# MichSchli/RelationPrediction

Hardware: AMD Instinct MI355X
Metric: processed edges/sec (R-GCN forward+backward), FB15k-237 gcn_block (higher is better)
Workload: dtype f32 (dense contractions: fp32 operands split exactly into 3 bf16, 6 of 9 partial products on the bf16 matrix cores, fp32 accumulation; error vs float64 equal to the fp32 MFMA's); 1 GPU; fb237_block; entities=14541, relations=237, dim=500, layers=2, kind=block, num_blocks_or_bases=100, graph_edges=15000, norm_mode=intended (1/deg of the edge's own row; SURVEY H1, DESIGN section 10), parallelism=single GPU

## Files before the change

### relationprediction_amd/csrc/block_msgs.hip

```cpp
#include <type_traits>

#include "rgcn_internal.h"

namespace rgcn {

namespace {

__device__ __forceinline__ int find_segment(const int32_t* __restrict__ ptr, int n_seg, int x) {
  int lo = 0, hi = n_seg;
  while (hi - lo > 1) {
    int mid = (lo + hi) >> 1;
    if (ptr[mid] <= x) lo = mid; else hi = mid;
  }
  return lo;
}

struct MsgArgs {
  const float* Hin;
  const float* D;
  const float* W;
  float* out;
  float* slab;
  const int32_t* m_src;
  const int32_t* m_dst;
  const int32_t* m_slot;
  const float* m_norm;
  const int32_t* rel_ptr;
  const int32_t* chunk_ptr;
  int32_t R2, nb, d, chunk, G;
};

template <int SD>
__global__ void k_block_msg_fwd(MsgArgs a) {
  const int bid = blockIdx.x;
  if (bid >= a.chunk_ptr[a.R2]) return;
  const int g = threadIdx.x / a.nb;
  if (g >= a.G) return;
  const int b = threadIdx.x - g * a.nb;
  const int rel = find_segment(a.chunk_ptr, a.R2, bid);
  const int beg = a.rel_ptr[rel] + (bid - a.chunk_ptr[rel]) * a.chunk;
  const int end = min(beg + a.chunk, a.rel_ptr[rel + 1]);
  float w[SD * SD];
#pragma unroll
  for (int k = 0; k < SD * SD; ++k) w[k] = a.W[((size_t)rel * SD * SD + k) * a.nb + b];
  const int col = b * SD;
// ... 4 lines not shown
    const float* xp = a.Hin + (size_t)src * a.d + col;
    float x[SD];
#pragma unroll
    for (int q = 0; q < SD; ++q) x[q] = xp[q];
    float* yp = a.out + (size_t)slot * a.d + col;
#pragma unroll
    for (int i = 0; i < SD; ++i) {
      float y = 0.0f;
#pragma unroll
      for (int q = 0; q < SD; ++q) y = fmaf(w[i * SD + q], x[q], y);
      yp[i] = y * nrm;
    }
  }
}

template <int SD, bool ZOUT>
__global__ void k_block_msg_bwd(MsgArgs a) {
  extern __shared__ float red[];
  const int bid = blockIdx.x;
  if (bid >= a.chunk_ptr[a.R2]) return;
  const int g = threadIdx.x / a.nb;
  const bool active = g < a.G;
  const int b = threadIdx.x - g * a.nb;
  const int rel = find_segment(a.chunk_ptr, a.R2, bid);
  const int beg = a.rel_ptr[rel] + (bid - a.chunk_ptr[rel]) * a.chunk;
  const int end = min(beg + a.chunk, a.rel_ptr[rel + 1]);
  float w[SD * SD], dw[SD * SD];
#pragma unroll
  for (int k = 0; k < SD * SD; ++k) dw[k] = 0.0f;
  if (active) {
    if constexpr (ZOUT) {
#pragma unroll
      for (int k = 0; k < SD * SD; ++k) w[k] = a.W[((size_t)rel * SD * SD + k) * a.nb + b];
    }
    const int col = b * SD;
    for (int j = beg + g; j < end; j += a.G) {
      const int src = a.m_src[j];
      const int dst = a.m_dst[j];
      const int slot = ZOUT ? a.m_slot[j] : 0;
      const float nrm = a.m_norm[j];
      const float* xp = a.Hin + (size_t)src * a.d + col;
      const float* gp = a.D + (size_t)dst * a.d + col;
      float x[SD], gr[SD];
#pragma unroll
      for (int q = 0; q < SD; ++q) { x[q] = xp[q]; gr[q] = gp[q] * nrm; }
      if constexpr (ZOUT) {
        float* zp = a.out + (size_t)slot * a.d + col;
#pragma unroll
        for (int q = 0; q < SD; ++q) {
          float z = 0.0f;
#pragma unroll
          for (int i = 0; i < SD; ++i) z = fmaf(w[i * SD + q], gr[i], z);
          zp[q] = z;
        }
      }
#pragma unroll
      for (int i = 0; i < SD; ++i)
#pragma unroll
        for (int q = 0; q < SD; ++q) dw[i * SD + q] = fmaf(gr[i], x[q], dw[i * SD + q]);
    }
  }
  if (a.G > 1) {
    if (active && g > 0) {
#pragma unroll
      for (int k = 0; k < SD * SD; ++k) red[((size_t)(g - 1) * SD * SD + k) * a.nb + b] = dw[k];
    }
    __syncthreads();
    if (active && g == 0) {
      for (int gg = 1; gg < a.G; ++gg)
#pragma unroll
        for (int k = 0; k < SD * SD; ++k) dw[k] += red[((size_t)(gg - 1) * SD * SD + k) * a.nb + b];
    }
  }
  if (active && g == 0) {
#pragma unroll
    for (int k = 0; k < SD * SD; ++k) a.slab[((size_t)bid * SD * SD + k) * a.nb + b] = dw[k];
  }
}

__global__ void k_block_dw_reduce(const float* __restrict__ slab, const int32_t* __restrict__ chunk_ptr,
                                  float* __restrict__ gW, int R2, int per_rel) {
  const int64_t i = (int64_t)blockIdx.x * blockDim.x + threadIdx.x;
  if (i >= (int64_t)R2 * per_rel) return;
  const int rel = (int)(i / per_rel);
  const int k = (int)(i - (int64_t)rel * per_rel);
  const int c0 = chunk_ptr[rel], c1 = chunk_ptr[rel + 1];
  float a0 = 0.f, a1 = 0.f, a2 = 0.f, a3 = 0.f, a4 = 0.f, a5 = 0.f, a6 = 0.f, a7 = 0.f;
  int c = c0;
  for (; c + 8 <= c1; c += 8) {
    const float* p = slab + (size_t)c * per_rel + k;
    a0 += p[0]; a1 += p[(size_t)per_rel]; a2 += p[2 * (size_t)per_rel]; a3 += p[3 * (size_t)per_rel];
    a4 += p[4 * (size_t)per_rel]; a5 += p[5 * (size_t)per_rel]; a6 += p[6 * (size_t)per_rel];
    a7 += p[7 * (size_t)per_rel];
  }
  for (; c < c1; ++c) a0 += slab[(size_t)c * per_rel + k];
  gW[i] = ((a0 + a1) + (a2 + a3)) + ((a4 + a5) + (a6 + a7));
}

__global__ void k_block_transpose(const float* __restrict__ in, float* __restrict__ out, int R, int nb,
                                  int sd2, int to_device) {
  const int64_t i = (int64_t)blockIdx.x * blockDim.x + threadIdx.x;
  const int64_t n = (int64_t)R * nb * sd2;
  if (i >= n) return;
  const int b = (int)(i % nb);
  const int k = (int)((i / nb) % sd2);
  const int r = (int)(i / ((int64_t)nb * sd2));
  const int64_t h = ((int64_t)r * nb + b) * sd2 + k;
  if (to_device) out[i] = in[h]; else out[h] = in[i];
}

int max_chunks(const rgcn_ctx* c) {
// ... 45 lines not shown
  a.rel_ptr = c->g.rel_ptr; a.chunk_ptr = c->g.chunk_ptr;
  a.R2 = 2 * c->R; a.nb = c->nb; a.d = c->d; a.chunk = c->g.chunk; a.G = c->msg_slots;
  const double M = 2.0 * c->g.E / c->world;
  const double rows = M < c->V ? M : (double)c->V;
  const double Wb = 8.0 * c->R * c->nb * c->sd * c->sd;
  ProfScope ps(c, "block_msg_fwd", M * (8.0 * c->d + 16.0) + Wb, M * 2.0 * c->d * c->sd,
               4.0 * c->d * (rows + M) + 16.0 * M + Wb);
  RGCN_TRY(dispatch_sd(c, [&](auto sdc) {
    constexpr int SD = decltype(sdc)::value;
    hipLaunchKernelGGL((k_block_msg_fwd<SD>), dim3(max_chunks(c)), dim3(c->msg_block), 0, c->stream, a);
  }));
  RGCN_HIP(c, hipGetLastError());
  return RGCN_OK;
}

rgcn_status block_msg_backward(rgcn_ctx* c, int layer, const float* Hin, const float* D, float* Zbuf) {
  const int per_rel = c->sd * c->sd * c->nb;
  const int R2 = 2 * c->R;
  if (c->g.E > 0) {
    const int nchunks = max_chunks(c);
    if ((size_t)nchunks * per_rel > c->slab_dw_floats)
      RGCN_FAIL(c, RGCN_ERR_STATE, "internal: dW slab buffer too small");
    MsgArgs a;
    a.Hin = Hin; a.D = D; a.W = c->layers[layer].wrel; a.out = Zbuf; a.slab = c->slab_dw;
    a.m_src = c->g.m_src; a.m_dst = c->g.m_dst; a.m_slot = c->g.m_sslot; a.m_norm = c->g.m_norm;
    a.rel_ptr = c->g.rel_ptr; a.chunk_ptr = c->g.chunk_ptr;
    a.R2 = R2; a.nb = c->nb; a.d = c->d; a.chunk = c->g.chunk; a.G = c->msg_slots;
    const size_t lds = (size_t)(c->msg_slots - 1) * per_rel * sizeof(float);
    const double M = 2.0 * c->g.E / c->world;
    const double rows = M < c->V ? M : (double)c->V;
    if (Zbuf != nullptr) {
      ProfScope ps(c, "block_msg_bwd", M * (12.0 * c->d + 20.0) + 16.0 * c->R * per_rel,
                   M * 4.0 * c->d * c->sd, 4.0 * c->d * (2.0 * rows + M) + 20.0 * M + 16.0 * c->R * per_rel);
      RGCN_TRY(dispatch_sd(c, [&](auto sdc) {
        constexpr int SD = decltype(sdc)::value;
        hipLaunchKernelGGL((k_block_msg_bwd<SD, true>), dim3(nchunks), dim3(c->msg_block), lds, c->stream, a);
      }));
    } else {
      ProfScope ps(c, "block_dw_msgs", M * (8.0 * c->d + 16.0) + 8.0 * c->R * per_rel, M * 2.0 * c->d * c->sd,
                   4.0 * c->d * 2.0 * rows + 16.0 * M + 8.0 * c->R * per_rel);
      RGCN_TRY(dispatch_sd(c, [&](auto sdc) {
        constexpr int SD = decltype(sdc)::value;
        hipLaunchKernelGGL((k_block_msg_bwd<SD, false>), dim3(nchunks), dim3(c->msg_block), lds, c->stream, a);
      }));
    }
    RGCN_HIP(c, hipGetLastError());
  }
  return RGCN_OK;
}

rgcn_status block_dw_reduce(rgcn_ctx* c, int layer) {
  const int per_rel = c->sd * c->sd * c->nb;
  const int R2 = 2 * c->R;
  {
    const int64_t n = (int64_t)R2 * per_rel;
    ProfScope ps(c, "block_dw_reduce", 8.0 * n, 0);
    hipLaunchKernelGGL(k_block_dw_reduce, dim3((unsigned)((n + 255) / 256)), dim3(256), 0, c->stream,
                       c->slab_dw, c->g.chunk_ptr, c->layers[layer].grel, R2, per_rel);
    RGCN_HIP(c, hipGetLastError());
  }
  return RGCN_OK;
}

rgcn_status block_to_device_layout(rgcn_ctx* c, const float* host_layout_dev, float* dst, int R) {
  const int64_t n = (int64_t)R * c->nb * c->sd * c->sd;
  hipLaunchKernelGGL(k_block_transpose, dim3((unsigned)((n + 255) / 256)), dim3(256), 0, c->stream,
                     host_layout_dev, dst, R, c->nb, c->sd * c->sd, 1);
  RGCN_HIP(c, hipGetLastError());
  return RGCN_OK;
}

rgcn_status block_from_device_layout(rgcn_ctx* c, const float* src, float* host_layout_dev, int R) {
  const int64_t n = (int64_t)R * c->nb * c->sd * c->sd;
  hipLaunchKernelGGL(k_block_transpose, dim3((unsigned)((n + 255) / 256)), dim3(256), 0, c->stream,
                     src, host_layout_dev, R, c->nb, c->sd * c->sd, 0);
// ... 6 lines not shown
```

### relationprediction_amd/csrc/graph_prep.hip

```cpp
#include "rgcn_internal.h"

namespace rgcn {

namespace {

constexpr int kScanThreads = 1024;
constexpr int kScanItems = 16;

struct ScanJob {
  const int32_t* in;
  int32_t* out;
  int32_t n;
  int32_t div;
  int32_t* where;
};
struct ScanJobs {
  ScanJob j[5];
};

__global__ void __launch_bounds__(kScanThreads) k_exscan(ScanJobs jobs) {
  const ScanJob job = jobs.j[blockIdx.x];
  __shared__ int32_t wsum[kScanThreads / 64];
  __shared__ int32_t carry_s;
  const int tid = threadIdx.x, lane = tid & 63, wid = tid >> 6;
// ... 66 lines not shown
}

__device__ __forceinline__ int lower_bound_u32(const uint32_t* a, int n, uint32_t x) {
  int lo = 0, hi = n;
  while (lo < hi) {
    int mid = (lo + hi) >> 1;
    if (a[mid] < x) lo = mid + 1; else hi = mid;
  }
  return lo;
}

__global__ void __launch_bounds__(1024) k_ptrs(const uint32_t* __restrict__ keyv_s,
                                               const uint32_t* __restrict__ keyr_s,
                                               const int32_t* __restrict__ permv, int E, int degrees_from_rows,
                                               int32_t* indeg, int32_t* outdeg, int M, int V, int R2,
                                               int chunk, int32_t* row_ptr,
                                               int32_t* long_rows, int32_t* nlong, int cap, int giant_threshold,
                                               int32_t* giant_rows, int32_t* giant_first, int32_t* giant_cnt,
                                               int32_t* piece_row, int32_t* piece_k, int32_t* ngiant, int giant_cap,
                                               int piece_cap, int32_t* rel_ptr, int32_t* chunk_ptr,
                                               uint32_t* row_key, int32_t* has_dir, uint32_t vmul) {
  if (blockIdx.x == 0) {
    __shared__ int32_t wsum[16];
    __shared__ int32_t carry_s;
    const int tid = threadIdx.x, lane = tid & 63, wid = tid >> 6;
    if (tid == 0) carry_s = 0;
    __syncthreads();
    for (int base = 0; base <= R2; base += 1024) {
      const int r = base + tid;
      int lo = 0, nchunks = 0;
      if (r <= R2) {
        lo = lower_bound_u32(keyr_s, M, (uint32_t)r);
        rel_ptr[r] = lo;
        if (r < R2) {
          const int hi = lower_bound_u32(keyr_s, M, (uint32_t)(r + 1));
          nchunks = (hi - lo + chunk - 1) / chunk;
        }
      }
      int incl = nchunks;
#pragma unroll
      for (int off = 1; off < 64; off <<= 1) {
        int t = __shfl_up(incl, off, 64);
        if (lane >= off) incl += t;
      }
      if (lane == 63) wsum[wid] = incl;
      __syncthreads();
      int wbase = 0, total = 0;
      for (int w = 0; w < 16; ++w) {
        if (w < wid) wbase += wsum[w];
        total += wsum[w];
      }
      const int carry = carry_s;
      if (r <= R2) chunk_ptr[r] = carry + wbase + incl - nchunks;
      __syncthreads();
      if (tid == 0) carry_s = carry + total;
      __syncthreads();
    }
    return;
  }
  const int v = (blockIdx.x - 1) * blockDim.x + threadIdx.x;
  if (v > V) return;
  const int beg = lower_bound_u32(keyv_s, M, (uint32_t)v * vmul);
  row_ptr[v] = beg;
  if (v == V) return;
  const int end = lower_bound_u32(keyv_s, M, (uint32_t)(v + 1) * vmul);
  if (row_key != nullptr) row_key[v] = end - beg > kLongRow ? (uint32_t)(kLongRow + 1) : (uint32_t)(kLongRow - (end - beg));
  if (degrees_from_rows || has_dir != nullptr) {
    int lo = beg, hi = end;
    while (lo < hi) {
      const int mid = (lo + hi) >> 1;
      if (permv[mid] < E) lo = mid + 1; else hi = mid;
// ... 226 lines not shown
  g.outdeg = g.counters + V;
  g.nlong = g.counters + 2 * V;
  g.ngiant = g.counters + 2 * V + 1;
  g.giant_cap = (int32_t)(M / kGiantRow + 1);
  g.piece_cap = (int32_t)(2 * (M / kGiantRow) + 2);
  RGCN_TRY(dalloc(c, &g.giant_rows, (size_t)g.giant_cap));
  RGCN_TRY(dalloc(c, &g.giant_first, (size_t)g.giant_cap));
  RGCN_TRY(dalloc(c, &g.giant_cnt, (size_t)g.giant_cap));
  RGCN_TRY(dalloc(c, &g.piece_row, (size_t)g.piece_cap));
  RGCN_TRY(dalloc(c, &g.piece_k, (size_t)g.piece_cap));
  g.long_cap = (int32_t)(M / kLongRow + 1);
  RGCN_TRY(dalloc(c, &g.long_rows, (size_t)g.long_cap));
  RGCN_TRY(dalloc(c, &g.row_ptr, V + 1));
  RGCN_TRY(dalloc(c, &g.rel_ptr, R2 + 1));
  RGCN_TRY(dalloc(c, &g.chunk_ptr, R2 + 1));
  RGCN_TRY(dalloc(c, &g.cum_in, V + 1));
  RGCN_TRY(dalloc(c, &g.cum_out, V + 1));
  RGCN_TRY(dalloc(c, &g.keyv, M));
  RGCN_TRY(dalloc(c, &g.keyv_s, M));
  RGCN_TRY(dalloc(c, &g.keyr, M));
  RGCN_TRY(dalloc(c, &g.keyr_s, M));
  RGCN_TRY(dalloc(c, &g.valv, M));
  RGCN_TRY(dalloc(c, &g.permv, M));
  RGCN_TRY(dalloc(c, &g.valr, M));
  RGCN_TRY(dalloc(c, &g.permr, M));
  RGCN_TRY(dalloc(c, &g.pos, M));
  RGCN_TRY(dalloc(c, &g.m_src, M));
  RGCN_TRY(dalloc(c, &g.m_dst, M));
  RGCN_TRY(dalloc(c, &g.m_dslot, M));
  RGCN_TRY(dalloc(c, &g.m_sslot, M));
// ... 20 lines not shown
  }
  if (share) {
    g.owner = share->owner;
    g.errflag = share->errflag;
  } else {
    RGCN_TRY(dalloc(c, &g.owner, (size_t)c->R));
    RGCN_TRY(dalloc(c, &g.errflag, 1));
    RGCN_HIP(c, hipMemsetAsync(g.owner, 0, sizeof(int32_t) * (size_t)(c->R ? c->R : 1), c->stream));
    RGCN_HIP(c, hipMemsetAsync(g.errflag, 0, sizeof(int32_t), c->stream));
  }
  RGCN_HIP(c, hipEventCreateWithFlags(&g.ev_ready, order_event_flags(c)));
  RGCN_HIP(c, hipEventCreateWithFlags(&g.ev_free, order_event_flags(c)));
  RGCN_HIP(c, hipMemsetAsync(g.row_ptr, 0, sizeof(int32_t) * (V + 1), c->stream));
  RGCN_HIP(c, hipMemsetAsync(g.rel_ptr, 0, sizeof(int32_t) * (R2 + 1), c->stream));
  RGCN_HIP(c, hipMemsetAsync(g.chunk_ptr, 0, sizeof(int32_t) * (R2 + 1), c->stream));
  RGCN_TRY(dalloc(c, &g.keyv_t, M));
  RGCN_TRY(dalloc(c, &g.keyr_t, M));
  RGCN_TRY(dalloc(c, &g.tablev, sort_table_elems(M)));
  RGCN_TRY(dalloc(c, &g.tabler, sort_table_elems(M)));
  return RGCN_OK;
}

static void graph_free_one(GraphBufs& g, bool owns_shared) {
  if (!owns_shared) { g.owner = nullptr; g.errflag = nullptr; }
  if (g.ev_ready) (void)hipEventDestroy(g.ev_ready);
  if (g.ev_free) (void)hipEventDestroy(g.ev_free);
  void* ptrs[] = {g.giant_rows, g.giant_first, g.giant_cnt, g.piece_row, g.piece_k, g.long_rows, g.triples, g.counters, g.row_ptr, g.rel_ptr, g.chunk_ptr, g.cum_in, g.cum_out,
                  g.keyv, g.keyv_s, g.keyr, g.keyr_s, g.valv, g.permv, g.valr, g.permr, g.pos,
                  g.m_src, g.m_dst, g.m_dslot, g.m_sslot, g.m_norm, g.d_src, g.d_rel, g.d_norm, g.s_dst, g.s_rel,
                  g.s_norm, g.owner, g.errflag, g.keyv_t, g.keyr_t, g.tablev, g.tabler, g.row_key, g.row_key_s, g.row_order,
                  g.row_tab, g.has_dir, g.unit_ptr, g.unit_rows};
  for (void* p : ptrs)
    if (p) (void)hipFree(p);
  g = GraphBufs();
}

void graph_free(rgcn_ctx* c) {
  graph_free_one(c->g_alt, false);
  graph_free_one(c->g, true);
}

rgcn_status graph_build(rgcn_ctx* c, const int32_t* tri, int64_t E64) {
  GraphBufs& g = c->g;
  const int E = (int)E64, V = c->V, R = c->R;
  const int M = 2 * E;
  g.cur = tri;
  g.E = E;
  g.chunk = std::min(c->chunk, 48 * (int)std::max<int64_t>(1, ((int64_t)M + 65535) / 65536));
  g.giant_on = c->kind == RGCN_KIND_BLOCK && c->world == 1 && M > 65536;
  g.ready = false;
  g.pf_valid = false;
  g.units_host = -1;
  c->fwd_done = false;
  const uint32_t vmul = (uint64_t)(V + 1) * (2 * (uint64_t)R) < (1ull << 31) ? (uint32_t)(2 * R) : 1u;
  const bool zero_in_keys = c->world == 1 && E > 0;
  if (!zero_in_keys) RGCN_HIP(c, hipMemsetAsync(g.counters, 0, g.counters_bytes, c->stream));
  const int T = 256;
  if (E > 0) {
    {
      ProfScope ps(c, "prep_keys", 12.0 * E + 16.0 * M, 0);
      hipLaunchKernelGGL(k_keys, dim3((M + T - 1) / T), dim3(T), 0, c->stream, tri, E, V, R, g.owner,
                         c->rank, g.keyv, g.keyr, c->world > 1 ? 1 : 0, g.indeg, g.outdeg, g.errflag,
                         zero_in_keys ? g.nlong : (int32_t*)nullptr, vmul);
    }
    SortSpec sp[2];
    sp[0] = SortSpec{g.keyv, g.keyv_s, g.permv, g.keyv_t, g.valv, g.pos, g.tablev, (int64_t)M, (uint32_t)V * vmul};
    sp[1] = SortSpec{g.keyr, g.keyr_s, g.permr, g.keyr_t, g.valr, nullptr, g.tabler, (int64_t)M, (uint32_t)(2 * R)};
    RGCN_TRY(sort_pairs(c, "prep_sort", 2, sp));
  }
  {
    ProfScope ps(c, "prep_ptrs", 8.0 * (V + 2 * R) + 4.0 * M, 0);
    hipLaunchKernelGGL(k_ptrs, dim3(1 + (V + 1 + 1023) / 1024), dim3(1024), 0, c->stream, g.keyv_s, g.keyr_s,
                       g.permv, E, c->world > 1 ? 0 : 1, g.indeg, g.outdeg, M, V, 2 * R, g.chunk, g.row_ptr, g.long_rows,
                       g.nlong, g.long_cap,
                       g.giant_on ? kGiantRow : 0x7fffffff, g.giant_rows, g.giant_first, g.giant_cnt, g.piece_row,
                       g.piece_k, g.ngiant, g.giant_cap, g.piece_cap, g.rel_ptr, g.chunk_ptr, g.row_key, g.has_dir, vmul);
  }
  if (g.row_key != nullptr) {
    SortSpec sp{g.row_key, g.row_key_s, g.row_order, g.row_key_s, g.row_order, nullptr, g.row_tab, (int64_t)V,
                (uint32_t)(kLongRow + 1)};
    RGCN_TRY(sort_pairs(c, "prep_row_order", 1, &sp));
  }
  {
    ScanJobs jobs;
    int nj = 0;
    if (c->cfg.norm_mode == RGCN_NORM_TF_AS_EXECUTED) {
      jobs.j[nj++] = {g.indeg, g.cum_in, V, 0, nullptr};
      jobs.j[nj++] = {g.outdeg, g.cum_out, V, 0, nullptr};
    }
    if (g.has_dir != nullptr) {
      jobs.j[nj++] = {g.has_dir, g.unit_ptr, V, 0, g.unit_rows};
// ... 45 lines not shown
```

### relationprediction_amd/csrc/rgcn_api.hip

```cpp
#include <cstdlib>
#include <mutex>
#include <utility>
#include <new>

#include "rgcn_api_internal.h"

namespace rgcn {

static std::mutex g_err_mu;
static std::string g_err;
void set_global_error(const std::string& s) {
  std::lock_guard<std::mutex> lk(g_err_mu);
  g_err = s;
}

ProfScope::ProfScope(rgcn_ctx* ctx, const char* name, double bytes, double flops, double compulsory) : c(ctx), idx(-1) {
  if (!c->prof_on) return;
  ProfRec r;
  r.name = name;
  r.bytes = bytes;
  r.flops = flops;
  r.cbytes = compulsory < 0 ? bytes : compulsory;
  for (int k = 0; k < 2; ++k) {
    hipEvent_t e = nullptr;
// ... 373 lines not shown
  add_param(c, "W_relation", {(int64_t)V, (int64_t)d}, c->w_rel, c->g_rel, LAYOUT_PLAIN);
  c->H.assign(c->L + 1, nullptr);
  for (int l = 0; l <= c->L; ++l) RGCN_TRY(dmalloc(c, &c->H[l], Vd));
  RGCN_TRY(dmalloc(c, &c->self_buf, Vd));
  if (c->world > 1) RGCN_TRY(dmalloc(c, &c->exch, Vd));
  for (int k = 0; k < 2; ++k) {
    RGCN_TRY(dmalloc(c, &c->dbuf[k], Vd));
    RGCN_TRY(dmalloc(c, &c->dsbuf[k], Vd));
  }
  const size_t M = 2 * (size_t)f.max_edges;
  size_t slab = 64 * d * d;
  const size_t max_rel_chunks = std::max((M + c->chunk - 1) / c->chunk, (std::min<size_t>(M, 65536) + 47) / 48) + 2 * R;
  if (c->kind == RGCN_KIND_BLOCK) {
    RGCN_TRY(dmalloc(c, &c->msgbuf, (M ? M : 1) * d, false));
    const size_t per_rel = (size_t)c->sd * c->sd * c->nb;
    c->slab_dw_floats = max_rel_chunks * per_rel;
    RGCN_TRY(dmalloc(c, &c->slab_dw, c->slab_dw_floats, false));
  } else {
    const size_t zc = 2 * (size_t)c->B * d;
    RGCN_TRY(dmalloc(c, &c->msgbuf2, V * zc));
    RGCN_TRY(dmalloc(c, &c->aggbuf, 2 * V * d));
    c->zsave.assign(c->L + 1, nullptr);
    for (int l = 1; l <= c->L; ++l) RGCN_TRY(dmalloc(c, &c->zsave[l], V * zc));
    const size_t s2 = 16 * zc * d;
    if (s2 > slab) slab = s2;
    c->slab_dw_floats = max_rel_chunks * (size_t)c->B;
    RGCN_TRY(dmalloc(c, &c->slab_dw, c->slab_dw_floats, false));
  }
  c->slab_floats = slab;
  RGCN_TRY(dmalloc(c, &c->slab, slab));
  size_t stage = Vd;
// ... 805 lines not shown
```

### relationprediction_amd/csrc/rgcn_internal.h

```cpp
#pragma once

#include <hip/hip_runtime.h>

#include <cstdint>
#include <cstdio>
#include <cstdlib>
#include <cstring>
#include <string>
#include <vector>

#include "../../include/rgcn.h"

namespace rgcn {

#ifdef RGCN_DEVTOOLS
inline int knob(const char* name, int dflt) {
  const char* s = getenv(name);
  return s ? atoi(s) : dflt;
}
#else
constexpr int knob(const char*, int dflt) { return dflt; }
#endif

void set_global_error(const std::string& s);
// ... 39 lines not shown
  const uint32_t hi = (uint32_t)(idx >> 32);
  uint32_t x = (uint32_t)idx ^ k.k0 ^ ((hi << 16) | (hi >> 16));
  x ^= x >> 16;
  x *= 0x7feb352du;
  x += k.k1;
  x ^= x >> 15;
  x *= 0x846ca68bu;
  x ^= x >> 16;
  return x >> 8;
}

enum DropMode { DROP_NONE = 0, DROP_RNG = 1, DROP_MASK = 2 };

constexpr int kLongRow = 32;
constexpr int kGiantRow = 2048;
constexpr int kAuxStreams = 3;

struct DropSpec {
  int32_t mode;
  uint32_t layer;
  uint32_t thresh;
  float inv_keep;
  uint64_t seed;
  const uint8_t* mask;
  const uint64_t* seed_offset;
};

#if defined(__HIPCC__)
__device__ __forceinline__ DropKey drop_key(const DropSpec& ds) {
  if (ds.mode != DROP_RNG) return DropKey{0u, 0u};
// ... 59 lines not shown
  size_t counters_bytes = 0;
  int32_t* row_ptr = nullptr;
  int32_t* long_rows = nullptr;
  int32_t *giant_rows = nullptr, *giant_first = nullptr, *giant_cnt = nullptr, *piece_row = nullptr, *piece_k = nullptr;
  int32_t* ngiant = nullptr;
  int32_t giant_cap = 0, piece_cap = 0;
  bool giant_on = false;
  uint32_t *row_key = nullptr, *row_key_s = nullptr;
  int32_t* row_order = nullptr;
  uint16_t* row_tab = nullptr;
  int32_t* nlong = nullptr;
  int32_t long_cap = 0;
  int32_t* rel_ptr = nullptr;
  int chunk = 48;
  int32_t* chunk_ptr = nullptr;
  int32_t* cum_in = nullptr;
  int32_t* cum_out = nullptr;
  uint32_t *keyv = nullptr, *keyv_s = nullptr, *keyr = nullptr, *keyr_s = nullptr;
  int32_t *valv = nullptr, *permv = nullptr, *valr = nullptr, *permr = nullptr;
  int32_t* pos = nullptr;
  int32_t *m_src = nullptr, *m_dst = nullptr, *m_dslot = nullptr, *m_sslot = nullptr;
  int32_t *d_src = nullptr, *d_rel = nullptr, *s_dst = nullptr, *s_rel = nullptr;
  float *d_norm = nullptr, *s_norm = nullptr;
  float* m_norm = nullptr;
  int32_t *has_dir = nullptr, *unit_ptr = nullptr, *unit_rows = nullptr;
  int64_t units_host = -1;
  uint32_t *keyv_t = nullptr, *keyr_t = nullptr;
  uint16_t *tablev = nullptr, *tabler = nullptr;
  const int32_t* pf_tri = nullptr;
  int64_t pf_E = -1;
// ... 239 lines not shown
rgcn_status gemm_presplit_b(rgcn_ctx* c, const PresplitJob* jobs, int n);

rgcn_status gemm_f32(rgcn_ctx* c, const char* tag, bool a_kc, bool b_kc, int M, int N, int K,
                     const float* A, int lda, const float* B, int ldb, float* C, int ldc,
                     int split_k, const GemmBatch* batch = nullptr, double prof_scale = 1.0);

hipError_t gemm_bf16x3_launch(rgcn_ctx* c, int terms, bool a_kc, bool b_kc, bool vec, int M, int N, int K,
                              const float* A, int lda, const float* B, int ldb, float* C, int ldc,
                              int k_per_split, int splits, int swizzle, int vecC, const GemmBatch* batch = nullptr);
hipError_t gemm_bf16x3_w8_launch(rgcn_ctx* c, int terms, int M, int N, int K, const float* A, int lda, float* C, int ldc,
                                 int swizzle, int vecC, const GemmBatch& batch);

rgcn_status block_geometry(rgcn_ctx* c);
rgcn_status block_msg_forward(rgcn_ctx* c, int layer, const float* Hin, float* Ybuf);
rgcn_status block_msg_backward(rgcn_ctx* c, int layer, const float* Hin, const float* D, float* Zbuf);
rgcn_status block_dw_reduce(rgcn_ctx* c, int layer);
rgcn_status block_to_device_layout(rgcn_ctx* c, const float* host_layout_dev, float* dst, int R);
rgcn_status block_from_device_layout(rgcn_ctx* c, const float* src, float* host_layout_dev, int R);

struct CombineArgs;
bool block_rows_available(const rgcn_ctx* c);
size_t block_rows_weight_floats(const rgcn_ctx* c);
rgcn_status block_rows(rgcn_ctx* c, const char* tag, int layer, bool backward, const float* X, const CombineArgs& ca);

rgcn_status basis_aggregate_forward(rgcn_ctx* c, int layer, const float* Hin, float* Z);
struct CombineArgs;
rgcn_status basis_backward_gather(rgcn_ctx* c, int layer, const float* dZ, const CombineArgs& ca,
                                  bool with_messages);
rgcn_status basis_dcoef(rgcn_ctx* c, int layer, const float* Hin, const float* dZ);
double basis_units(rgcn_ctx* c);
// ... 74 lines not shown
```

### relationprediction_amd/csrc/rgcn_schedule.hip

```cpp
#include "rgcn_api_internal.h"

namespace rgcn {

rgcn_status fwd_begin(rgcn_ctx* c, int train, uint64_t seed, const uint8_t* masks_host) {
  if (!c->g.ready) RGCN_FAIL(c, RGCN_ERR_STATE, "rgcn_forward before rgcn_set_graph");
  RGCN_TRY(join_abandoned_side_work(c));
  c->fwd_done = false;
  c->frag_fresh = false;
  c->wtile_fresh = false;
  c->fwd_train = train ? 1 : 0;
  c->seed = seed;
  c->explicit_masks = false;
  if (train && masks_host) {
    const size_t n = (size_t)c->L * c->V * c->d;
    if (!c->masks) RGCN_TRY(dmalloc(c, &c->masks, n, false));
    RGCN_TRY(to_dev(c, c->masks, masks_host, n));
    c->explicit_masks = true;
  }
  return input_forward(c);
}

static rgcn_status wait_gather(rgcn_ctx* c) {
  if (c->gather_pending) {
    RGCN_HIP(c, hipStreamWaitEvent(c->stream, c->ev_gather, 0));
// ... 188 lines not shown
  auto self_dh = [&]() {
    return gemm_f32(c, "gemm_self_dh", true, true, rows, d, d, c->bwd_dS + (size_t)lo * d, d, lb.wself, d,
                    c->self_buf + (size_t)lo * d, d, 1, &sbt);
  };
  bool defer_joins = false;
  if (c->kind == RGCN_KIND_BLOCK && rows_layer(c)) {
    const bool minibatch = c->world == 1 && c->g.E <= 65536;
    if (minibatch && c->use_aux) {
      {
        StreamScope side(c, 1);
        RGCN_TRY(self_dw());
      }
      RGCN_TRY(self_dh());
      {
        StreamScope side(c, 0);
        RGCN_TRY(block_msg_backward(c, l, Hin, c->bwd_D, nullptr));
        RGCN_TRY(block_dw_reduce(c, l));
      }
      RGCN_TRY(block_rows(c, "block_rows_bwd", l, true, c->bwd_D, a));
      defer_joins = l == 2;
      if (!defer_joins) RGCN_TRY(stream_join_both(c));
    } else if (minibatch) {
      RGCN_TRY(block_msg_backward(c, l, Hin, c->bwd_D, nullptr));
      {
        StreamScope side(c, 1, true);
        RGCN_TRY(block_dw_reduce(c, l));
        RGCN_TRY(self_dw());
      }
      RGCN_TRY(self_dh());
      RGCN_TRY(block_rows(c, "block_rows_bwd", l, true, c->bwd_D, a));
    } else {
      {
        StreamScope side(c, 0);
        RGCN_TRY(wait_gather(c));
        RGCN_TRY(block_msg_backward(c, l, Hin, c->bwd_D, nullptr));
        RGCN_TRY(block_dw_reduce(c, l));
        c->dw_pending = side.active;
      }
      {
        StreamScope side(c, 1);
        RGCN_TRY(self_dw());
      }
      RGCN_TRY(self_dh());
      RGCN_TRY(wait_gather(c));
      RGCN_TRY(block_rows(c, "block_rows_bwd", l, true, c->bwd_D, a));
    }
  } else if (c->kind == RGCN_KIND_BLOCK) {
    {
      StreamScope side(c, 0);
      RGCN_TRY(wait_gather(c));
      RGCN_TRY(block_msg_backward(c, l, Hin, c->bwd_D, c->msgbuf));
      if (side.active) RGCN_HIP(c, hipEventRecord(c->ev_join[0], c->aux[0]));
      RGCN_TRY(block_dw_reduce(c, l));
    }
    RGCN_TRY(self_dh());
    {
      StreamScope side(c, 1);
      RGCN_TRY(self_dw());
    }
    if (c->use_aux) RGCN_HIP(c, hipStreamWaitEvent(c->main_stream, c->ev_join[0], 0));
    a.msg = c->g.E > 0 ? c->msgbuf : nullptr;
    a.row_ptr = c->g.row_ptr;
    a.long_rows = c->g.long_rows;
    a.nlong = c->g.nlong;
    RGCN_TRY(combine(c, "combine_bwd", a, 4.0 * d * ((a.out2 ? 4.0 : 3.0) * V + Mmsg) + 4.0 * V));
  } else {
    const int Bd = c->B * d;
// ... 116 lines not shown
```

Measured before the change: 29.63 million edges/s.

## Split block dW into partitioned kernel with direct writes for small relations

Moves the block-diagonal weight-gradient computation into its own kernel that splits edges by a new per-relation partition size (part_ptr built during graph prep). Relations with few edges write their gradient straight into gW, and only larger relations go through the partial-sum slab and reduce, which now launches as a 2D grid per relation. The dW loop adds float4 vector loads and prefetches indices two iterations ahead. In the fused Z+dW path the message backward is split into two kernels, so Hin/D rows are read twice there. The slab buffer is sized by the new partition cap.

```diff
diff --git a/relationprediction_amd/csrc/block_msgs.hip b/relationprediction_amd/csrc/block_msgs.hip
--- a/relationprediction_amd/csrc/block_msgs.hip
+++ b/relationprediction_amd/csrc/block_msgs.hip
@@ -21,14 +21,34 @@
   const float* W;
   float* out;
   float* slab;
+  float* gW;
   const int32_t* m_src;
   const int32_t* m_dst;
   const int32_t* m_slot;
   const float* m_norm;
   const int32_t* rel_ptr;
   const int32_t* chunk_ptr;
+  const int32_t* part_ptr;
   int32_t R2, nb, d, chunk, G;
+  int32_t part, part_cap;
 };
+
+template <int SD>
+__device__ __forceinline__ void load_piece(const float* __restrict__ p, float (&v)[SD]) {
+  if constexpr (SD % 4 == 0) {
+#pragma unroll
+    for (int k = 0; k < SD / 4; ++k) {
+      const float4 t = reinterpret_cast<const float4*>(p)[k];
+      v[4 * k] = t.x; v[4 * k + 1] = t.y; v[4 * k + 2] = t.z; v[4 * k + 3] = t.w;
+    }
+  } else if constexpr (SD == 2) {
+    const float2 t = *reinterpret_cast<const float2*>(p);
+    v[0] = t.x; v[1] = t.y;
+  } else {
+#pragma unroll
+    for (int q = 0; q < SD; ++q) v[q] = p[q];
+  }
+}
 
 template <int SD>
 __global__ void k_block_msg_fwd(MsgArgs a) {
@@ -63,50 +83,99 @@
   }
 }
 
-template <int SD, bool ZOUT>
-__global__ void k_block_msg_bwd(MsgArgs a) {
-  extern __shared__ float red[];
+template <int SD>
+__device__ __forceinline__ void msg_rows_bwd(const MsgArgs& a) {
   const int bid = blockIdx.x;
   if (bid >= a.chunk_ptr[a.R2]) return;
   const int g = threadIdx.x / a.nb;
-  const bool active = g < a.G;
+  if (g >= a.G) return;
   const int b = threadIdx.x - g * a.nb;
   const int rel = find_segment(a.chunk_ptr, a.R2, bid);
   const int beg = a.rel_ptr[rel] + (bid - a.chunk_ptr[rel]) * a.chunk;
   const int end = min(beg + a.chunk, a.rel_ptr[rel + 1]);
-  float w[SD * SD], dw[SD * SD];
+  float w[SD * SD];
+#pragma unroll
+  for (int k = 0; k < SD * SD; ++k) w[k] = a.W[((size_t)rel * SD * SD + k) * a.nb + b];
+  const int col = b * SD;
+  for (int j = beg + g; j < end; j += a.G) {
+    const int dst = a.m_dst[j];
+    const int slot = a.m_slot[j];
+    const float nrm = a.m_norm[j];
+    const float* gp = a.D + (size_t)dst * a.d + col;
+    float gr[SD];
+#pragma unroll
+    for (int q = 0; q < SD; ++q) gr[q] = gp[q] * nrm;
+    float* zp = a.out + (size_t)slot * a.d + col;
+#pragma unroll
+    for (int q = 0; q < SD; ++q) {
+      float z = 0.0f;
+#pragma unroll
+      for (int i = 0; i < SD; ++i) z = fmaf(w[i * SD + q], gr[i], z);
+      zp[q] = z;
+    }
+  }
+}
+
+constexpr int kInFlight = 2;
+
+template <int SD>
+__device__ __forceinline__ void rel_weight_grad(const MsgArgs& a) {
+  extern __shared__ float red[];
+  constexpr int U = kInFlight;
+  const int bid = blockIdx.x;
+  int beg, end;
+  float* out;
+  if (bid < a.part_cap) {
+    if (bid >= a.part_ptr[a.R2]) return;
+    const int rel = find_segment(a.part_ptr, a.R2, bid);
+    beg = a.rel_ptr[rel] + (bid - a.part_ptr[rel]) * a.part;
+    end = min(beg + a.part, a.rel_ptr[rel + 1]);
+    out = a.slab + (size_t)bid * SD * SD * a.nb;
+  } else {
+    const int rel = bid - a.part_cap;
+    beg = a.rel_ptr[rel];
+    end = a.rel_ptr[rel + 1];
+    if (end - beg > a.part) return;
+    out = a.gW + (size_t)rel * SD * SD * a.nb;
+  }
+  const int g = threadIdx.x / a.nb;
+  const bool active = g < a.G;
+  const int b = threadIdx.x - g * a.nb;
+  float dw[SD * SD];
 #pragma unroll
   for (int k = 0; k < SD * SD; ++k) dw[k] = 0.0f;
-  if (active) {
-    if constexpr (ZOUT) {
-#pragma unroll
-      for (int k = 0; k < SD * SD; ++k) w[k] = a.W[((size_t)rel * SD * SD + k) * a.nb + b];
-    }
-    const int col = b * SD;
-    for (int j = beg + g; j < end; j += a.G) {
-      const int src = a.m_src[j];
-      const int dst = a.m_dst[j];
-      const int slot = ZOUT ? a.m_slot[j] : 0;
-      const float nrm = a.m_norm[j];
-      const float* xp = a.Hin + (size_t)src * a.d + col;
-      const float* gp = a.D + (size_t)dst * a.d + col;
-      float x[SD], gr[SD];
-#pragma unroll
-      for (int q = 0; q < SD; ++q) { x[q] = xp[q]; gr[q] = gp[q] * nrm; }
-      if constexpr (ZOUT) {
-        float* zp = a.out + (size_t)slot * a.d + col;
-#pragma unroll
-        for (int q = 0; q < SD; ++q) {
-          float z = 0.0f;
-#pragma unroll
-          for (int i = 0; i < SD; ++i) z = fmaf(w[i * SD + q], gr[i], z);
-          zp[q] = z;
+  if (active && beg + g < end) {
+    const int col = b * SD, G = a.G;
+    int src[U], dst[U];
+    float nrm[U];
+    auto fetch_indices = [&](int j0) {
+#pragma unroll
+      for (int u = 0; u < U; ++u) {
+        const int j = min(j0 + u * G, end - 1);
+        src[u] = a.m_src[j]; dst[u] = a.m_dst[j]; nrm[u] = a.m_norm[j];
+      }
+    };
+    fetch_indices(beg + g);
+    for (int j0 = beg + g; j0 < end; j0 += U * G) {
+      float x[U][SD], gr[U][SD], n[U];
+#pragma unroll
+      for (int u = 0; u < U; ++u) {
+        load_piece<SD>(a.Hin + (size_t)src[u] * a.d + col, x[u]);
+        load_piece<SD>(a.D + (size_t)dst[u] * a.d + col, gr[u]);
+        n[u] = nrm[u];
+      }
+      if (j0 + U * G < end) fetch_indices(j0 + U * G);
+#pragma unroll
+      for (int u = 0; u < U; ++u) {
+        if (j0 + u * G < end) {
+#pragma unroll
+          for (int i = 0; i < SD; ++i) {
+            const float gi = gr[u][i] * n[u];
+#pragma unroll
+            for (int q = 0; q < SD; ++q) dw[i * SD + q] = fmaf(gi, x[u][q], dw[i * SD + q]);
+          }
         }
       }
-#pragma unroll
-      for (int i = 0; i < SD; ++i)
-#pragma unroll
-        for (int q = 0; q < SD; ++q) dw[i * SD + q] = fmaf(gr[i], x[q], dw[i * SD + q]);
     }
   }
   if (a.G > 1) {
@@ -123,17 +192,22 @@
   }
   if (active && g == 0) {
 #pragma unroll
-    for (int k = 0; k < SD * SD; ++k) a.slab[((size_t)bid * SD * SD + k) * a.nb + b] = dw[k];
-  }
-}
-
-__global__ void k_block_dw_reduce(const float* __restrict__ slab, const int32_t* __restrict__ chunk_ptr,
-                                  float* __restrict__ gW, int R2, int per_rel) {
-  const int64_t i = (int64_t)blockIdx.x * blockDim.x + threadIdx.x;
-  if (i >= (int64_t)R2 * per_rel) return;
-  const int rel = (int)(i / per_rel);
-  const int k = (int)(i - (int64_t)rel * per_rel);
-  const int c0 = chunk_ptr[rel], c1 = chunk_ptr[rel + 1];
+    for (int k = 0; k < SD * SD; ++k) out[(size_t)k * a.nb + b] = dw[k];
+  }
+}
+
+template <int SD, bool ZOUT>
+__global__ void __launch_bounds__(512) k_block_msg_bwd(MsgArgs a) {
+  if constexpr (ZOUT) msg_rows_bwd<SD>(a); else rel_weight_grad<SD>(a);
+}
+
+__global__ void k_block_dw_reduce(const float* __restrict__ slab, const int32_t* __restrict__ part_ptr,
+                                  float* __restrict__ gW, int per_rel) {
+  const int rel = blockIdx.x;
+  const int c0 = part_ptr[rel], c1 = part_ptr[rel + 1];
+  if (c0 == c1) return;
+  const int k = blockIdx.y * blockDim.x + threadIdx.x;
+  if (k >= per_rel) return;
   float a0 = 0.f, a1 = 0.f, a2 = 0.f, a3 = 0.f, a4 = 0.f, a5 = 0.f, a6 = 0.f, a7 = 0.f;
   int c = c0;
   for (; c + 8 <= c1; c += 8) {
@@ -143,7 +217,7 @@
     a7 += p[7 * (size_t)per_rel];
   }
   for (; c < c1; ++c) a0 += slab[(size_t)c * per_rel + k];
-  gW[i] = ((a0 + a1) + (a2 + a3)) + ((a4 + a5) + (a6 + a7));
+  gW[(size_t)rel * per_rel + k] = ((a0 + a1) + (a2 + a3)) + ((a4 + a5) + (a6 + a7));
 }
 
 __global__ void k_block_transpose(const float* __restrict__ in, float* __restrict__ out, int R, int nb,
@@ -219,51 +293,58 @@
   return RGCN_OK;
 }
 
+static MsgArgs backward_args(rgcn_ctx* c, int layer, const float* Hin, const float* D, float* Zbuf) {
+  MsgArgs a;
+  a.Hin = Hin; a.D = D; a.W = c->layers[layer].wrel; a.out = Zbuf; a.slab = c->slab_dw; a.gW = c->layers[layer].grel;
+  a.m_src = c->g.m_src; a.m_dst = c->g.m_dst; a.m_slot = c->g.m_sslot; a.m_norm = c->g.m_norm;
+  a.rel_ptr = c->g.rel_ptr; a.chunk_ptr = c->g.chunk_ptr; a.part_ptr = c->g.part_ptr;
+  a.R2 = 2 * c->R; a.nb = c->nb; a.d = c->d; a.chunk = c->g.chunk; a.G = c->msg_slots;
+  a.part = c->g.part; a.part_cap = dw_part_cap(2 * (int64_t)c->g.E, a.R2);
+  return a;
+}
+
 rgcn_status block_msg_backward(rgcn_ctx* c, int layer, const float* Hin, const float* D, float* Zbuf) {
+  if (c->g.E == 0) return RGCN_OK;
+  const MsgArgs a = backward_args(c, layer, Hin, D, Zbuf);
   const int per_rel = c->sd * c->sd * c->nb;
-  const int R2 = 2 * c->R;
-  if (c->g.E > 0) {
-    const int nchunks = max_chunks(c);
-    if ((size_t)nchunks * per_rel > c->slab_dw_floats)
-      RGCN_FAIL(c, RGCN_ERR_STATE, "internal: dW slab buffer too small");
-    MsgArgs a;
-    a.Hin = Hin; a.D = D; a.W = c->layers[layer].wrel; a.out = Zbuf; a.slab = c->slab_dw;
-    a.m_src = c->g.m_src; a.m_dst = c->g.m_dst; a.m_slot = c->g.m_sslot; a.m_norm = c->g.m_norm;
-    a.rel_ptr = c->g.rel_ptr; a.chunk_ptr = c->g.chunk_ptr;
-    a.R2 = R2; a.nb = c->nb; a.d = c->d; a.chunk = c->g.chunk; a.G = c->msg_slots;
-    const size_t lds = (size_t)(c->msg_slots - 1) * per_rel * sizeof(float);
-    const double M = 2.0 * c->g.E / c->world;
-    const double rows = M < c->V ? M : (double)c->V;
-    if (Zbuf != nullptr) {
-      ProfScope ps(c, "block_msg_bwd", M * (12.0 * c->d + 20.0) + 16.0 * c->R * per_rel,
-                   M * 4.0 * c->d * c->sd, 4.0 * c->d * (2.0 * rows + M) + 20.0 * M + 16.0 * c->R * per_rel);
-      RGCN_TRY(dispatch_sd(c, [&](auto sdc) {
-        constexpr int SD = decltype(sdc)::value;
-        hipLaunchKernelGGL((k_block_msg_bwd<SD, true>), dim3(nchunks), dim3(c->msg_block), lds, c->stream, a);
-      }));
-    } else {
-      ProfScope ps(c, "block_dw_msgs", M * (8.0 * c->d + 16.0) + 8.0 * c->R * per_rel, M * 2.0 * c->d * c->sd,
-                   4.0 * c->d * 2.0 * rows + 16.0 * M + 8.0 * c->R * per_rel);
-      RGCN_TRY(dispatch_sd(c, [&](auto sdc) {
-        constexpr int SD = decltype(sdc)::value;
-        hipLaunchKernelGGL((k_block_msg_bwd<SD, false>), dim3(nchunks), dim3(c->msg_block), lds, c->stream, a);
-      }));
-    }
-    RGCN_HIP(c, hipGetLastError());
-  }
+  const double M = 2.0 * c->g.E / c->world;
+  const double rows = M < c->V ? M : (double)c->V;
+  ProfScope ps(c, "block_msg_bwd", M * (8.0 * c->d + 12.0) + 8.0 * c->R * per_rel, M * 2.0 * c->d * c->sd,
+               4.0 * c->d * (rows + M) + 12.0 * M + 8.0 * c->R * per_rel);
+  RGCN_TRY(dispatch_sd(c, [&](auto sdc) {
+    constexpr int SD = decltype(sdc)::value;
+    hipLaunchKernelGGL((k_block_msg_bwd<SD, true>), dim3(max_chunks(c)), dim3(c->msg_block), 0, c->stream, a);
+  }));
+  RGCN_HIP(c, hipGetLastError());
+  return RGCN_OK;
+}
+
+rgcn_status block_dw_msgs(rgcn_ctx* c, int layer, const float* Hin, const float* D) {
+  const MsgArgs a = backward_args(c, layer, Hin, D, nullptr);
+  const int per_rel = c->sd * c->sd * c->nb;
+  if ((size_t)a.part_cap * per_rel > c->slab_dw_floats)
+    RGCN_FAIL(c, RGCN_ERR_STATE, "internal: dW partial-sum buffer too small");
+  const size_t lds = (size_t)(c->msg_slots - 1) * per_rel * sizeof(float);
+  const double M = 2.0 * c->g.E / c->world;
+  const double rows = M < c->V ? M : (double)c->V;
+  ProfScope ps(c, "block_dw_msgs", M * (8.0 * c->d + 12.0) + 8.0 * c->R * per_rel, M * 2.0 * c->d * c->sd,
+               4.0 * c->d * 2.0 * rows + 12.0 * M + 8.0 * c->R * per_rel);
+  RGCN_TRY(dispatch_sd(c, [&](auto sdc) {
+    constexpr int SD = decltype(sdc)::value;
+    hipLaunchKernelGGL((k_block_msg_bwd<SD, false>), dim3(a.part_cap + a.R2), dim3(c->msg_block), lds, c->stream, a);
+  }));
+  RGCN_HIP(c, hipGetLastError());
   return RGCN_OK;
 }
 
 rgcn_status block_dw_reduce(rgcn_ctx* c, int layer) {
+  if (c->g.E == 0) return RGCN_OK;
   const int per_rel = c->sd * c->sd * c->nb;
-  const int R2 = 2 * c->R;
-  {
-    const int64_t n = (int64_t)R2 * per_rel;
-    ProfScope ps(c, "block_dw_reduce", 8.0 * n, 0);
-    hipLaunchKernelGGL(k_block_dw_reduce, dim3((unsigned)((n + 255) / 256)), dim3(256), 0, c->stream,
-                       c->slab_dw, c->g.chunk_ptr, c->layers[layer].grel, R2, per_rel);
-    RGCN_HIP(c, hipGetLastError());
-  }
+  const double parts = (double)(2 * (int64_t)c->g.E / c->g.part);
+  ProfScope ps(c, "block_dw_reduce", 4.0 * per_rel * (parts + std::min<double>(parts, 2.0 * c->R)), 0);
+  hipLaunchKernelGGL(k_block_dw_reduce, dim3(2 * c->R, (per_rel + 255) / 256), dim3(256), 0, c->stream, c->slab_dw,
+                     c->g.part_ptr, c->layers[layer].grel, per_rel);
+  RGCN_HIP(c, hipGetLastError());
   return RGCN_OK;
 }
 
diff --git a/relationprediction_amd/csrc/graph_prep.hip b/relationprediction_amd/csrc/graph_prep.hip
--- a/relationprediction_amd/csrc/graph_prep.hip
+++ b/relationprediction_amd/csrc/graph_prep.hip
@@ -104,47 +104,52 @@
                                                const uint32_t* __restrict__ keyr_s,
                                                const int32_t* __restrict__ permv, int E, int degrees_from_rows,
                                                int32_t* indeg, int32_t* outdeg, int M, int V, int R2,
-                                               int chunk, int32_t* row_ptr,
+                                               int chunk, int part, int32_t* row_ptr,
                                                int32_t* long_rows, int32_t* nlong, int cap, int giant_threshold,
                                                int32_t* giant_rows, int32_t* giant_first, int32_t* giant_cnt,
                                                int32_t* piece_row, int32_t* piece_k, int32_t* ngiant, int giant_cap,
                                                int piece_cap, int32_t* rel_ptr, int32_t* chunk_ptr,
-                                               uint32_t* row_key, int32_t* has_dir, uint32_t vmul) {
+                                               int32_t* part_ptr, uint32_t* row_key, int32_t* has_dir, uint32_t vmul) {
   if (blockIdx.x == 0) {
     __shared__ int32_t wsum[16];
-    __shared__ int32_t carry_s;
+    __shared__ int32_t carry_s[2];
     const int tid = threadIdx.x, lane = tid & 63, wid = tid >> 6;
-    if (tid == 0) carry_s = 0;
+    if (tid < 2) carry_s[tid] = 0;
     __syncthreads();
     for (int base = 0; base <= R2; base += 1024) {
       const int r = base + tid;
-      int lo = 0, nchunks = 0;
+      int lo = 0, cnt[2] = {0, 0};
       if (r <= R2) {
         lo = lower_bound_u32(keyr_s, M, (uint32_t)r);
         rel_ptr[r] = lo;
         if (r < R2) {
-          const int hi = lower_bound_u32(keyr_s, M, (uint32_t)(r + 1));
-          nchunks = (hi - lo + chunk - 1) / chunk;
+          const int n = lower_bound_u32(keyr_s, M, (uint32_t)(r + 1)) - lo;
+          cnt[0] = (n + chunk - 1) / chunk;
+          cnt[1] = n > part ? (n + part - 1) / part : 0;
         }
       }
-      int incl = nchunks;
-#pragma unroll
-      for (int off = 1; off < 64; off <<= 1) {
-        int t = __shfl_up(incl, off, 64);
-        if (lane >= off) incl += t;
-      }
-      if (lane == 63) wsum[wid] = incl;
-      __syncthreads();
-      int wbase = 0, total = 0;
-      for (int w = 0; w < 16; ++w) {
-        if (w < wid) wbase += wsum[w];
-        total += wsum[w];
-      }
-      const int carry = carry_s;
-      if (r <= R2) chunk_ptr[r] = carry + wbase + incl - nchunks;
-      __syncthreads();
-      if (tid == 0) carry_s = carry + total;
-      __syncthreads();
+#pragma unroll
+      for (int s = 0; s < 2; ++s) {
+        int32_t* out = s == 0 ? chunk_ptr : part_ptr;
+        int incl = cnt[s];
+#pragma unroll
+        for (int off = 1; off < 64; off <<= 1) {
+          int t = __shfl_up(incl, off, 64);
+          if (lane >= off) incl += t;
+        }
+        if (lane == 63) wsum[wid] = incl;
+        __syncthreads();
+        int wbase = 0, total = 0;
+        for (int w = 0; w < 16; ++w) {
+          if (w < wid) wbase += wsum[w];
+          total += wsum[w];
+        }
+        const int carry = carry_s[s];
+        if (r <= R2) out[r] = carry + wbase + incl - cnt[s];
+        __syncthreads();
+        if (tid == 0) carry_s[s] = carry + total;
+        __syncthreads();
+      }
     }
     return;
   }
@@ -401,6 +406,7 @@
   RGCN_TRY(dalloc(c, &g.row_ptr, V + 1));
   RGCN_TRY(dalloc(c, &g.rel_ptr, R2 + 1));
   RGCN_TRY(dalloc(c, &g.chunk_ptr, R2 + 1));
+  RGCN_TRY(dalloc(c, &g.part_ptr, R2 + 1));
   RGCN_TRY(dalloc(c, &g.cum_in, V + 1));
   RGCN_TRY(dalloc(c, &g.cum_out, V + 1));
   RGCN_TRY(dalloc(c, &g.keyv, M));
@@ -451,6 +457,7 @@
   RGCN_HIP(c, hipMemsetAsync(g.row_ptr, 0, sizeof(int32_t) * (V + 1), c->stream));
   RGCN_HIP(c, hipMemsetAsync(g.rel_ptr, 0, sizeof(int32_t) * (R2 + 1), c->stream));
   RGCN_HIP(c, hipMemsetAsync(g.chunk_ptr, 0, sizeof(int32_t) * (R2 + 1), c->stream));
+  RGCN_HIP(c, hipMemsetAsync(g.part_ptr, 0, sizeof(int32_t) * (R2 + 1), c->stream));
   RGCN_TRY(dalloc(c, &g.keyv_t, M));
   RGCN_TRY(dalloc(c, &g.keyr_t, M));
   RGCN_TRY(dalloc(c, &g.tablev, sort_table_elems(M)));
@@ -462,7 +469,7 @@
   if (!owns_shared) { g.owner = nullptr; g.errflag = nullptr; }
   if (g.ev_ready) (void)hipEventDestroy(g.ev_ready);
   if (g.ev_free) (void)hipEventDestroy(g.ev_free);
-  void* ptrs[] = {g.giant_rows, g.giant_first, g.giant_cnt, g.piece_row, g.piece_k, g.long_rows, g.triples, g.counters, g.row_ptr, g.rel_ptr, g.chunk_ptr, g.cum_in, g.cum_out,
+  void* ptrs[] = {g.giant_rows, g.giant_first, g.giant_cnt, g.piece_row, g.piece_k, g.long_rows, g.triples, g.counters, g.row_ptr, g.rel_ptr, g.chunk_ptr, g.part_ptr, g.cum_in, g.cum_out,
                   g.keyv, g.keyv_s, g.keyr, g.keyr_s, g.valv, g.permv, g.valr, g.permr, g.pos,
                   g.m_src, g.m_dst, g.m_dslot, g.m_sslot, g.m_norm, g.d_src, g.d_rel, g.d_norm, g.s_dst, g.s_rel,
                   g.s_norm, g.owner, g.errflag, g.keyv_t, g.keyr_t, g.tablev, g.tabler, g.row_key, g.row_key_s, g.row_order,
@@ -484,6 +491,7 @@
   g.cur = tri;
   g.E = E;
   g.chunk = std::min(c->chunk, 48 * (int)std::max<int64_t>(1, ((int64_t)M + 65535) / 65536));
+  g.part = dw_part_size(M);
   g.giant_on = c->kind == RGCN_KIND_BLOCK && c->world == 1 && M > 65536;
   g.ready = false;
   g.pf_valid = false;
@@ -508,10 +516,10 @@
   {
     ProfScope ps(c, "prep_ptrs", 8.0 * (V + 2 * R) + 4.0 * M, 0);
     hipLaunchKernelGGL(k_ptrs, dim3(1 + (V + 1 + 1023) / 1024), dim3(1024), 0, c->stream, g.keyv_s, g.keyr_s,
-                       g.permv, E, c->world > 1 ? 0 : 1, g.indeg, g.outdeg, M, V, 2 * R, g.chunk, g.row_ptr, g.long_rows,
+                       g.permv, E, c->world > 1 ? 0 : 1, g.indeg, g.outdeg, M, V, 2 * R, g.chunk, g.part, g.row_ptr, g.long_rows,
                        g.nlong, g.long_cap,
                        g.giant_on ? kGiantRow : 0x7fffffff, g.giant_rows, g.giant_first, g.giant_cnt, g.piece_row,
-                       g.piece_k, g.ngiant, g.giant_cap, g.piece_cap, g.rel_ptr, g.chunk_ptr, g.row_key, g.has_dir, vmul);
+                       g.piece_k, g.ngiant, g.giant_cap, g.piece_cap, g.rel_ptr, g.chunk_ptr, g.part_ptr, g.row_key, g.has_dir, vmul);
   }
   if (g.row_key != nullptr) {
     SortSpec sp{g.row_key, g.row_key_s, g.row_order, g.row_key_s, g.row_order, nullptr, g.row_tab, (int64_t)V,
diff --git a/relationprediction_amd/csrc/rgcn_api.hip b/relationprediction_amd/csrc/rgcn_api.hip
--- a/relationprediction_amd/csrc/rgcn_api.hip
+++ b/relationprediction_amd/csrc/rgcn_api.hip
@@ -411,7 +411,7 @@
   if (c->kind == RGCN_KIND_BLOCK) {
     RGCN_TRY(dmalloc(c, &c->msgbuf, (M ? M : 1) * d, false));
     const size_t per_rel = (size_t)c->sd * c->sd * c->nb;
-    c->slab_dw_floats = max_rel_chunks * per_rel;
+    c->slab_dw_floats = std::max<size_t>(1, (size_t)dw_part_cap_any((int64_t)M, 2 * (int64_t)R)) * per_rel;
     RGCN_TRY(dmalloc(c, &c->slab_dw, c->slab_dw_floats, false));
   } else {
     const size_t zc = 2 * (size_t)c->B * d;
diff --git a/relationprediction_amd/csrc/rgcn_internal.h b/relationprediction_amd/csrc/rgcn_internal.h
--- a/relationprediction_amd/csrc/rgcn_internal.h
+++ b/relationprediction_amd/csrc/rgcn_internal.h
@@ -2,6 +2,7 @@
 
 #include <hip/hip_runtime.h>
 
+#include <algorithm>
 #include <cstdint>
 #include <cstdio>
 #include <cstdlib>
@@ -77,6 +78,17 @@
 
 constexpr int kLongRow = 32;
 constexpr int kGiantRow = 2048;
+constexpr int kDwPart = 40;
+constexpr int kDwPartSpan = 131072;
+inline int dw_part_size(int64_t M) { return kDwPart * (int)std::max<int64_t>(1, (M + kDwPartSpan - 1) / kDwPartSpan); }
+inline int dw_part_cap(int64_t M, int64_t R2) {
+  const int64_t whole = M / dw_part_size(M);
+  return (int)(whole + std::min(R2, whole));
+}
+inline int dw_part_cap_any(int64_t M, int64_t R2) {
+  const int64_t whole = std::min<int64_t>(M, kDwPartSpan) / kDwPart;
+  return (int)(whole + std::min(R2, whole));
+}
 constexpr int kAuxStreams = 3;
 
 struct DropSpec {
@@ -166,6 +178,8 @@
   int32_t* rel_ptr = nullptr;
   int chunk = 48;
   int32_t* chunk_ptr = nullptr;
+  int part = kDwPart;
+  int32_t* part_ptr = nullptr;
   int32_t* cum_in = nullptr;
   int32_t* cum_out = nullptr;
   uint32_t *keyv = nullptr, *keyv_s = nullptr, *keyr = nullptr, *keyr_s = nullptr;
@@ -435,6 +449,7 @@
 rgcn_status block_geometry(rgcn_ctx* c);
 rgcn_status block_msg_forward(rgcn_ctx* c, int layer, const float* Hin, float* Ybuf);
 rgcn_status block_msg_backward(rgcn_ctx* c, int layer, const float* Hin, const float* D, float* Zbuf);
+rgcn_status block_dw_msgs(rgcn_ctx* c, int layer, const float* Hin, const float* D);
 rgcn_status block_dw_reduce(rgcn_ctx* c, int layer);
 rgcn_status block_to_device_layout(rgcn_ctx* c, const float* host_layout_dev, float* dst, int R);
 rgcn_status block_from_device_layout(rgcn_ctx* c, const float* src, float* host_layout_dev, int R);
diff --git a/relationprediction_amd/csrc/rgcn_schedule.hip b/relationprediction_amd/csrc/rgcn_schedule.hip
--- a/relationprediction_amd/csrc/rgcn_schedule.hip
+++ b/relationprediction_amd/csrc/rgcn_schedule.hip
@@ -226,14 +226,14 @@
       RGCN_TRY(self_dh());
       {
         StreamScope side(c, 0);
-        RGCN_TRY(block_msg_backward(c, l, Hin, c->bwd_D, nullptr));
+        RGCN_TRY(block_dw_msgs(c, l, Hin, c->bwd_D));
         RGCN_TRY(block_dw_reduce(c, l));
       }
       RGCN_TRY(block_rows(c, "block_rows_bwd", l, true, c->bwd_D, a));
       defer_joins = l == 2;
       if (!defer_joins) RGCN_TRY(stream_join_both(c));
     } else if (minibatch) {
-      RGCN_TRY(block_msg_backward(c, l, Hin, c->bwd_D, nullptr));
+      RGCN_TRY(block_dw_msgs(c, l, Hin, c->bwd_D));
       {
         StreamScope side(c, 1, true);
         RGCN_TRY(block_dw_reduce(c, l));
@@ -245,7 +245,7 @@
       {
         StreamScope side(c, 0);
         RGCN_TRY(wait_gather(c));
-        RGCN_TRY(block_msg_backward(c, l, Hin, c->bwd_D, nullptr));
+        RGCN_TRY(block_dw_msgs(c, l, Hin, c->bwd_D));
         RGCN_TRY(block_dw_reduce(c, l));
         c->dw_pending = side.active;
       }
@@ -263,6 +263,7 @@
       RGCN_TRY(wait_gather(c));
       RGCN_TRY(block_msg_backward(c, l, Hin, c->bwd_D, c->msgbuf));
       if (side.active) RGCN_HIP(c, hipEventRecord(c->ev_join[0], c->aux[0]));
+      RGCN_TRY(block_dw_msgs(c, l, Hin, c->bwd_D));
       RGCN_TRY(block_dw_reduce(c, l));
     }
     RGCN_TRY(self_dh());
```

Result: no change. 29.88 million edges/s, median of 6 (+0.8%).
